# AaltoML/free-hunch

Measured on AMD Instinct MI355X. Metric: images/sec (256x256, num_steps=30, FH-Heun), higher is better.
Workload: dtype f32 UNet (convolutions: exact 3-way bf16 split on the bf16 MFMA, fp32 accuracy) + f64 covariance/CG; 1 GPU; FFHQ-256 arch, gaussian_blur, FH low-rank covariance (dct_diagonal), num_steps=30 heun, batch=8 per GPU; lockstep_groups_per_gpu=2, unet_backend=hip, net_calls_per_image=59

## Files before the change

### free-hunch_amd/_lib.py

```python
from __future__ import annotations

import ctypes as C
import os

import torch

_HERE = os.path.dirname(os.path.abspath(__file__))
LIB_PATH = os.path.join(_HERE, "libfh_hip.so")

c_dp = C.c_void_p


class FhProblem(C.Structure):
    _fields_ = [("op", C.c_int32), ("use_dct", C.c_int32), ("planes", C.c_int32), ("stride", C.c_int32),
                ("ntaps", C.c_int32), ("m", C.c_int32), ("ldm", C.c_int32), ("halo", C.c_int32),
                ("d", C.c_int64), ("sigma_y2", C.c_double),
                ("tap_dy", c_dp), ("tap_dx", c_dp), ("tap_w", c_dp), ("mask", c_dp),
                ("D", c_dp), ("r", c_dp), ("B", c_dp), ("M", c_dp),
                ("ntaps2", C.c_int32), ("halo2", C.c_int32), ("cg_scipy", C.c_int32), ("fold_sym", C.c_int32),
                ("tap2_dy", c_dp), ("tap2_dx", c_dp), ("tap2_w", c_dp),
                ("fold_fwd_w", c_dp), ("fold_fwd_h", c_dp), ("fold_inv_w", c_dp), ("fold_inv_h", c_dp)]


FH_MAX_BATCH = 16
# ... 19 lines not shown
    _fields_ = [("niter", C.c_int32), ("optimal", C.c_int32), ("residual_norm", C.c_double),
                ("b_norm", C.c_double)]


_SIGS = {
    "fh_version": ([], C.c_int),
    "fh_context_create": ([C.POINTER(C.c_void_p), C.c_int, C.c_int, C.c_int], C.c_int),
    "fh_context_destroy": ([C.c_void_p], C.c_int),
    "fh_context_set_exclusive": ([C.c_void_p, C.c_int], C.c_int),
    "fh_context_status": ([C.c_void_p, C.c_void_p], C.c_int),
    "fh_debug_read_stamps": ([C.c_void_p, C.POINTER(C.c_ulonglong), C.c_int, C.c_void_p], C.c_int),
    "fh_dct2d": ([C.c_void_p, c_dp, c_dp, C.c_int, C.c_int, C.c_void_p], C.c_int),
    "fh_dct_sym_plan": ([C.c_int, C.c_int] + [C.POINTER(C.c_int)] * 4 + [C.POINTER(C.c_int64)], C.c_int),
    "fh_dct_rect": ([C.c_void_p, c_dp, c_dp, c_dp, c_dp, C.c_int, C.c_int, C.c_int, C.c_void_p], C.c_int),
    "fh_dct_rect_plan": ([C.c_int] * 4 + [C.POINTER(C.c_int32)], C.c_int),
    "fh_dct_moments_u8": ([C.c_void_p, c_dp, C.c_int, c_dp, c_dp, c_dp, C.c_void_p], C.c_int),
    "fh_rep_apply": ([C.c_void_p, c_dp, c_dp, c_dp, c_dp, C.c_int, c_dp, c_dp, C.c_int64, C.c_int, C.c_void_p], C.c_int),
    "fh_rep_apply_batched": ([C.c_void_p, C.POINTER(FhBatch), C.c_int, c_dp, c_dp, C.c_int64, C.c_int, C.c_void_p], C.c_int),
    "fh_rep_invert": ([C.c_void_p, c_dp, c_dp, c_dp, C.c_double, c_dp, c_dp, c_dp, C.c_int, C.c_int64, C.c_int,
                       C.c_void_p], C.c_int),
    "fh_space_prep": ([C.c_void_p, c_dp, C.c_double, c_dp, c_dp, c_dp, C.c_int64, C.c_void_p], C.c_int),
    "fh_dot": ([C.c_void_p, c_dp, c_dp, c_dp, C.c_int, C.c_int64, C.c_void_p], C.c_int),
    "fh_space_commit": ([C.c_void_p, c_dp, c_dp, C.c_double, C.c_double, C.c_double, c_dp, c_dp, c_dp, c_dp, c_dp,
                         c_dp, c_dp, c_dp, C.c_int, C.c_int64, C.c_void_p], C.c_int),
    "fh_space_commit_dev": ([C.c_void_p, c_dp, c_dp, c_dp, C.c_double, c_dp, c_dp, c_dp, c_dp, c_dp, c_dp, c_dp, c_dp,
                             c_dp, C.c_int, C.c_int, c_dp, C.c_int, C.c_int, C.c_int, C.c_int64, C.c_void_p], C.c_int),
    "fh_cov_time_update": ([C.c_void_p, C.POINTER(FhCovState), c_dp, c_dp, C.c_double, C.c_double, C.c_double, C.c_int,
                            c_dp, c_dp, c_dp, c_dp, C.c_void_p], C.c_int),
    "fh_cov_space_update": ([C.c_void_p, C.POINTER(FhCovState), c_dp, c_dp, C.c_double, c_dp, c_dp, C.c_void_p], C.c_int),
    "fh_cov_time_update_batched": ([C.c_void_p, C.c_int, C.POINTER(FhCovState), c_dp, c_dp, C.c_double, C.c_double, C.c_double,
                                    c_dp, c_dp, c_dp, C.c_void_p], C.c_int),
    "fh_cov_space_update_batched": ([C.c_void_p, C.c_int, C.POINTER(FhCovState), c_dp, c_dp, C.c_double, c_dp, c_dp, c_dp,
                                     C.c_void_p], C.c_int),
    "fh_woodbury_inner": ([C.c_void_p, c_dp, C.c_int, c_dp, C.c_int, c_dp, C.c_int, C.c_int, C.c_void_p], C.c_int),
    "fh_axpby": ([C.c_double, c_dp, C.c_double, c_dp, c_dp, C.c_int64, C.c_void_p], C.c_int),
    "fh_read_scalars": ([C.c_void_p, c_dp, C.POINTER(C.c_double), C.c_int, C.c_void_p], C.c_int),
    "fh_conv_circ": ([C.c_void_p, c_dp, c_dp, c_dp, c_dp, c_dp, C.c_int, C.c_int, C.c_int, C.c_int, C.c_int,
                      C.c_void_p], C.c_int),
    "fh_conv_circ_plan": ([C.c_int] * 6 + [C.POINTER(C.c_int32)], C.c_int),
    "fh_conv_window": ([C.c_void_p, c_dp, c_dp, c_dp, C.c_int, C.c_int, C.c_int, C.c_int, C.c_void_p], C.c_int),
    "fh_conv_window_plan": ([C.c_int] * 4 + [C.POINTER(C.c_int32)], C.c_int),
    "fh_channel_mix": ([C.c_void_p, c_dp, c_dp, c_dp, C.c_int, C.c_int, C.c_void_p], C.c_int),
    "fh_amm": ([C.c_void_p, C.POINTER(FhProblem), c_dp, c_dp, C.c_void_p], C.c_int),
    "fh_dense_matvec_scratch_doubles": ([C.c_int, C.c_int64], C.c_int64),
    "fh_dense_matvec": ([c_dp, c_dp, c_dp, c_dp, C.c_int, C.c_int64, C.c_int, C.c_double, C.c_double, C.c_void_p], C.c_int),
    "fh_dense_rank2": ([c_dp, c_dp, C.c_int, C.c_int64, c_dp, c_dp, c_dp, c_dp, c_dp, c_dp, C.c_double, C.c_double,
                        C.c_void_p], C.c_int),
    "fh_conv2d_nhwc": ([c_dp, c_dp, c_dp, c_dp, c_dp, c_dp] + [C.c_int] * 10 + [C.c_void_p], C.c_int),
    "fh_conv2d_x6_nhwc": ([c_dp, c_dp, c_dp, c_dp, c_dp, c_dp] + [C.c_int] * 10 + [C.c_void_p], C.c_int),
    "fh_conv2d_x6_nhwc_gn": ([c_dp, c_dp, c_dp, c_dp, c_dp, c_dp] + [C.c_int] * 10 + [C.POINTER(FhGnEpilogue), C.c_void_p],
                             C.c_int),
    "fh_conv2d_x6_gn_chunks": ([C.c_int] * 10, C.c_int),
    "fh_conv2d_x6_plan": ([C.c_int] * 10 + [C.POINTER(C.c_int32)], C.c_int),
    "fh_groupnorm_finalize": ([c_dp, c_dp, C.c_int, C.c_int, C.c_double, C.c_int, C.c_void_p], C.c_int),
    "fh_groupnorm_bwd_table": ([c_dp, c_dp, c_dp, c_dp, c_dp, C.c_int, c_dp, C.c_int, C.c_int, C.c_void_p], C.c_int),
    "fh_groupnorm_bwd_apply": ([c_dp] * 8 + [C.c_int, c_dp] + [C.c_int] * 5 + [C.c_void_p], C.c_int),
    "fh_groupnorm_bwd_sums": ([c_dp] * 7 + [C.c_int, c_dp, c_dp] + [C.c_int] * 4 + [C.c_void_p], C.c_int),
    "fh_groupnorm_bwd_apply_ex": ([c_dp] * 8 + [C.c_int, c_dp, c_dp, c_dp, c_dp] + [C.c_int] * 5 + [c_dp, C.c_void_p], C.c_int),
    "fh_groupnorm_small_supported": ([C.c_int, C.c_int], C.c_int),
    "fh_groupnorm_fwd_small": ([c_dp] * 5 + [C.c_int, c_dp, c_dp] + [C.c_int] * 4 + [C.c_void_p], C.c_int),
    "fh_groupnorm_bwd_small": ([c_dp] * 8 + [C.c_int, c_dp, c_dp, c_dp, c_dp] + [C.c_int] * 5 + [C.c_void_p], C.c_int),
    "fh_conv2d_splitk": ([C.c_int] * 7, C.c_int),
    "fh_unet_set_precision": ([C.c_int], C.c_int),
    "fh_unet_get_precision": ([], C.c_int),
    "fh_absmax_f32": ([c_dp, C.c_int64, c_dp, C.c_void_p], C.c_int),
    "fh_groupnorm_table": ([c_dp, c_dp, c_dp, c_dp, c_dp, C.c_int, c_dp, C.c_int, C.c_int, C.c_void_p], C.c_int),
    "fh_conv2d_x6_norm_supported": ([C.c_int] * 5, C.c_int),
    "fh_conv2d_x6_norm_nhwc": ([c_dp, c_dp, C.c_int, c_dp, c_dp, c_dp, c_dp] + [C.c_int] * 5 + [C.c_void_p], C.c_int),
    "fh_conv2d_x6_norm_nhwc_gn": ([c_dp, c_dp, C.c_int, c_dp, c_dp, c_dp, c_dp] + [C.c_int] * 5
                                  + [C.POINTER(FhGnEpilogue), C.c_void_p], C.c_int),
    "fh_conv3x3_thin_nhwc": ([c_dp, c_dp, c_dp, c_dp] + [C.c_int] * 5 + [C.c_void_p], C.c_int),
    "fh_conv3x3_wino_nhwc": ([c_dp, c_dp, c_dp, c_dp, c_dp] + [C.c_int] * 5 + [C.c_void_p], C.c_int),
    "fh_bgemm_f32": ([c_dp, c_dp, c_dp] + [C.c_int] * 10 + [C.c_int64] * 6 + [C.c_float, C.c_void_p], C.c_int),
    "fh_groupnorm_scratch_doubles": ([C.c_int, C.c_int], C.c_int64),
    "fh_groupnorm_stats": ([c_dp, c_dp, c_dp, C.c_int, C.c_int, C.c_int, C.c_void_p], C.c_int),
    "fh_groupnorm_apply": ([c_dp] * 6 + [C.c_int, c_dp, C.c_int, C.c_int, C.c_int, C.c_int, C.c_void_p], C.c_int),
    "fh_groupnorm_bwd": ([c_dp] * 7 + [C.c_int, c_dp, c_dp, c_dp] + [C.c_int] * 5 + [C.c_void_p], C.c_int),
    "fh_attention_supported": ([C.c_int] * 3, C.c_int),
    "fh_attention_fwd": ([c_dp, c_dp, c_dp] + [C.c_int] * 5 + [C.c_void_p], C.c_int),
    "fh_attention_bwd": ([c_dp] * 6 + [C.c_int] * 5 + [C.c_void_p], C.c_int),
    "fh_softmax_rows": ([c_dp, C.c_int64, C.c_int, C.c_void_p], C.c_int),
    "fh_softmax_bwd_rows": ([c_dp, c_dp, C.c_int64, C.c_int, C.c_void_p], C.c_int),
    "fh_resample2x": ([c_dp, c_dp] + [C.c_int] * 5 + [C.c_void_p], C.c_int),
    "fh_concat_channels": ([c_dp, c_dp, c_dp, C.c_int64, C.c_int, C.c_int, C.c_int, C.c_void_p], C.c_int),
    "fh_layout_nchw_nhwc": ([c_dp, c_dp, C.c_int, C.c_int, C.c_int64, C.c_int, C.c_int, C.c_void_p], C.c_int),
    "fh_add_f32": ([c_dp, c_dp, c_dp, C.c_int64, C.c_void_p], C.c_int),
    "fh_metrics_scratch_doubles": ([C.c_int] * 4, C.c_int64),
    "fh_metrics_u8": ([c_dp, c_dp, C.c_int, C.c_int, C.c_int, C.c_int, c_dp, c_dp, c_dp, C.c_void_p], C.c_int),
    "fh_lpips_prep_u8": ([c_dp, c_dp, c_dp, c_dp, C.c_int, C.c_int, C.c_int, C.c_void_p], C.c_int),
    "fh_relu_f32": ([c_dp, C.c_int64, C.c_void_p], C.c_int),
    "fh_relu_maxpool2_nhwc": ([c_dp, c_dp, C.c_int, C.c_int, C.c_int, C.c_int, C.c_void_p], C.c_int),
    "fh_lpips_tap_scratch_doubles": ([C.c_int], C.c_int64),
    "fh_lpips_tap": ([c_dp, c_dp, C.c_int, C.c_int, C.c_int, C.c_int, c_dp, c_dp, C.c_int, C.c_void_p], C.c_int),
    "fh_noisy_u8": ([c_dp, C.POINTER(C.c_int64), C.c_int, C.c_int, C.c_double, C.c_int, C.c_uint64, c_dp, C.c_void_p], C.c_int),
    "fh_sqerr_u8_scratch_doubles": ([C.c_int, C.c_int], C.c_int64),
    "fh_sqerr_u8": ([c_dp, c_dp, C.c_int, C.c_int, c_dp, c_dp, C.c_void_p], C.c_int),
    "fh_cg_solve_batched": ([C.c_void_p, C.POINTER(FhProblem), C.POINTER(FhBatch), c_dp, c_dp, C.POINTER(C.c_double),
                             C.c_double, C.c_int, C.POINTER(FhCgInfo), C.c_void_p], C.c_int),
    "fh_cg_solve": ([C.c_void_p, C.POINTER(FhProblem), c_dp, c_dp, C.c_double, C.c_double, C.c_int,
                     C.POINTER(FhCgInfo), C.c_void_p], C.c_int),
}

_lib = None


class FhError(RuntimeError):
# ... 134 lines not shown
```

### free-hunch_amd/csrc/fh_unet.hip

```cpp
#include "fh_common.h"
#include <stdlib.h>

typedef float float16_t __attribute__((ext_vector_type(16)));

namespace {

constexpr int kBK = 32;
constexpr int kLd = kBK + 4;

struct ConvArgs {
  const float* in;
  const float* w;
  const float* bias;
  const float* res;
  float* out;
  int N, H, W, Cin, Cout, KH, KW, pad, stride, Ho, Wo;
  int ksplit;
  float* ws;
};

__device__ __forceinline__ void xcd_tile(int& tile_m, int& tile_n) {
  const unsigned gx = gridDim.x, gy = gridDim.y;
  const unsigned total = gx * gy;
  unsigned lin = blockIdx.y * gx + blockIdx.x;
// ... 235 lines not shown
    a.gn_partial[((int64_t)n * a.gn_chunks + chunk) * 64 + tid] = sum;
  }
}

__device__ __forceinline__ void split3(float x, __bf16& h, __bf16& m, __bf16& l) {
  h = (__bf16)x;
  float r = x - (float)h;
  m = (__bf16)r;
  r -= (float)m;
  l = (__bf16)r;
}

typedef _Float16 f16x8_t __attribute__((ext_vector_type(8)));
__device__ __forceinline__ __bf16 half_bits(float x) {
  const _Float16 h = (_Float16)x;
  return __builtin_bit_cast(__bf16, h);
}
template <bool F16>
__device__ __forceinline__ float16_t mfma16(bf16x8_t a, bf16x8_t b, float16_t c) {
  if (F16) return __builtin_amdgcn_mfma_f32_32x32x16_f16(__builtin_bit_cast(f16x8_t, a), __builtin_bit_cast(f16x8_t, b), c, 0, 0, 0);
  return __builtin_amdgcn_mfma_f32_32x32x16_bf16(a, b, c, 0, 0, 0);
}

struct SplitScale {
  float in, inv_in, winv;
};
template <int NP, bool F16>
__device__ __forceinline__ SplitScale split_scale(const ConvArgsX& a, int64_t wplane) {
  SplitScale s{1.f, 1.f, 1.f};
  if (F16 && NP == 2) {
    s.winv = *reinterpret_cast<const float*>(a.wx + 2 * wplane);
    if (a.in_amax != nullptr) {
      unsigned mb = 0u;
#pragma unroll
      for (int q = 0; q < FH_AMAX_SLOTS; ++q) mb = max(mb, __float_as_uint(a.in_amax[q]));
      int e = (int)((mb >> 23) & 255u) - 127;
      e = e < -110 ? -110 : (e > 126 ? 126 : e);
      s.in = __uint_as_float((unsigned)(127 + 11 - e) << 23);
      s.inv_in = __uint_as_float((unsigned)(127 - 11 + e) << 23);
    } else {
      s.in = a.in_scale;
      s.inv_in = 1.f / a.in_scale;
    }
  }
  return s;
}
__device__ __forceinline__ void split_half2(float xs, __bf16& h, __bf16& m) {
  xs = fminf(fmaxf(xs, -65504.f), 65504.f);
  const _Float16 hh = (_Float16)xs;
  h = __builtin_bit_cast(__bf16, hh);
  m = half_bits(xs - (float)hh);
}

template <int MI, int NI, int WM, int WN, int MINW, int NP = 3, bool F16 = false>
__global__ __launch_bounds__(64 * WM * WN, MINW) void k_conv_x6(ConvArgsX a) {
  constexpr int T = 64 * WM * WN;
  constexpr int BM = WM * MI * 32, BN = WN * NI * 32;
  constexpr int IA = BM * 8 / T;
  constexpr int IB = (NP * BN * 4 + T - 1) / T;
  static_assert(BM * 8 % T == 0, "tile / thread-count mismatch");
  __shared__ __align__(16) __bf16 As[NP][BM][kXLd];
  __shared__ __align__(16) __bf16 Bs[NP][BN][kXLd];

  const int tid = threadIdx.x, lane = tid & 63, wave = tid >> 6;
  const int wm = (wave / WN) * (MI * 32), wn = (wave % WN) * (NI * 32);
  const int lr = lane & 31, lh = lane >> 5;
  const int64_t M = (int64_t)a.N * a.Ho * a.Wo;
  int tile_m, tile_n;
  xcd_tile(tile_m, tile_n);
  const int64_t m0 = (int64_t)tile_m * BM;
  const int n0 = tile_n * BN;
  const int taps = a.KH * a.KW;
  const int cpt = a.Cin / kBK;
  const int nchunks_all = taps * cpt;
  const int c_begin = (int)((int64_t)nchunks_all * blockIdx.z / a.ksplit);
  const int c_end = (int)((int64_t)nchunks_all * (blockIdx.z + 1) / a.ksplit);

  int a_row[IA], a_n[IA], a_ho[IA], a_wo[IA];
  bool a_ok[IA];
  const int a_c4 = (tid & 7) * 4;
#pragma unroll
  for (int e = 0; e < IA; ++e) {
    a_row[e] = (e * T + tid) >> 3;
    const int64_t pm = m0 + a_row[e];
    a_ok[e] = pm < M;
    a_n[e] = a_ho[e] = a_wo[e] = 0;
    if (a_ok[e]) {
      a_n[e] = (int)(pm / ((int64_t)a.Ho * a.Wo));
      const int rem = (int)(pm % ((int64_t)a.Ho * a.Wo));
      a_ho[e] = rem / a.Wo;
      a_wo[e] = rem % a.Wo;
    }
  }
  const int64_t wplane = (int64_t)taps * cpt * a.Cout * kBK;
  const SplitScale ssc = split_scale<NP, F16>(a, wplane);
  int b_pl[IB], b_row[IB];
  bool b_ok[IB];
  const int b_part = (tid & 3) * 8;
#pragma unroll
  for (int e = 0; e < IB; ++e) {
    const int idx = e * T + tid;
    b_pl[e] = idx < NP * BN * 4 ? idx / (BN * 4) : -1;
    b_row[e] = (idx % (BN * 4)) >> 2;
    b_ok[e] = b_pl[e] >= 0 && n0 + b_row[e] < a.Cout;
  }

  float4 ra_reg[IA];
  bf16x8_t rb_reg[IB];

  auto load_chunk = [&](int c) {
    const int cc = c / taps, tap = c % taps;
    const int ky = tap / a.KW, kx = tap % a.KW;
#pragma unroll
    for (int e = 0; e < IA; ++e) {
      const int hi = a_ho[e] * a.stride + ky - a.pad, wi = a_wo[e] * a.stride + kx - a.pad;
      const bool ok = a_ok[e] && hi >= 0 && hi < a.H && wi >= 0 && wi < a.W;
      const float* src = a.in + (((int64_t)a_n[e] * a.H + (ok ? hi : 0)) * a.W + (ok ? wi : 0)) * a.Cin + cc * kBK + a_c4;
      ra_reg[e] = ok ? *reinterpret_cast<const float4*>(src) : make_float4(0.f, 0.f, 0.f, 0.f);
    }
    const __bf16* wbase = a.wx + ((int64_t)tap * cpt + cc) * a.Cout * kBK;
#pragma unroll
    for (int e = 0; e < IB; ++e) {
      bf16x8_t z;
#pragma unroll
      for (int q = 0; q < 8; ++q) z[q] = (__bf16)0.f;
      const __bf16* src = wbase + (b_ok[e] ? b_pl[e] : 0) * wplane + (int64_t)(b_ok[e] ? n0 + b_row[e] : 0) * kBK + b_part;
      rb_reg[e] = b_ok[e] ? *reinterpret_cast<const bf16x8_t*>(src) : z;
    }
  };
  typedef __bf16 bf16x4_t __attribute__((ext_vector_type(4)));
  auto store_chunk = [&]() {
#pragma unroll
    for (int e = 0; e < IA; ++e) {
      bf16x4_t h4, m4, l4;
      const float4 v = ra_reg[e];
#pragma unroll
      for (int q = 0; q < 4; ++q) {
        const float x = q == 0 ? v.x : q == 1 ? v.y : q == 2 ? v.z : v.w;
        __bf16 h, m, l;
        if (F16 && NP == 2) {
          split_half2(x * ssc.in, h, m);
          l = m;
        } else {
          split3(x, h, m, l);
          if (F16) h = half_bits(x);
        }
        h4[q] = h, m4[q] = m, l4[q] = l;
      }
      *reinterpret_cast<bf16x4_t*>(&As[0][a_row[e]][a_c4]) = h4;
      if (NP >= 2) *reinterpret_cast<bf16x4_t*>(&As[NP >= 2 ? 1 : 0][a_row[e]][a_c4]) = m4;
      if (NP == 3) *reinterpret_cast<bf16x4_t*>(&As[NP - 1][a_row[e]][a_c4]) = l4;
    }
#pragma unroll
    for (int e = 0; e < IB; ++e)
      if (b_pl[e] >= 0) *reinterpret_cast<bf16x8_t*>(&Bs[b_pl[e]][b_row[e]][b_part]) = rb_reg[e];
  };

  float16_t acc[MI][NI];
#pragma unroll
  for (int i = 0; i < MI; ++i)
#pragma unroll
    for (int j = 0; j < NI; ++j)
#pragma unroll
      for (int r = 0; r < 16; ++r) acc[i][j][r] = 0.f;

  auto compute = [&]() {
#pragma unroll
  for (int ks = 0; ks < kBK / 16; ++ks) {
    const int ko = ks * 16 + 8 * lh;
    bf16x8_t af[NP][MI], bfr[NP][NI];
#pragma unroll
    for (int p = 0; p < NP; ++p) {
#pragma unroll
      for (int i = 0; i < MI; ++i) af[p][i] = *reinterpret_cast<const bf16x8_t*>(&As[p][wm + i * 32 + lr][ko]);
#pragma unroll
      for (int j = 0; j < NI; ++j) bfr[p][j] = *reinterpret_cast<const bf16x8_t*>(&Bs[p][wn + j * 32 + lr][ko]);
    }
#pragma unroll
    for (int i = 0; i < MI; ++i)
#pragma unroll
      for (int j = 0; j < NI; ++j) {
        float16_t t = acc[i][j];
        if (NP == 3) {
          t = __builtin_amdgcn_mfma_f32_32x32x16_bf16(af[NP - 1][i], bfr[0][j], t, 0, 0, 0);
          t = __builtin_amdgcn_mfma_f32_32x32x16_bf16(af[0][i], bfr[NP - 1][j], t, 0, 0, 0);
          t = __builtin_amdgcn_mfma_f32_32x32x16_bf16(af[NP >= 2 ? 1 : 0][i], bfr[NP >= 2 ? 1 : 0][j], t, 0, 0, 0);
        }
        if (NP >= 2) {
          t = mfma16<F16>(af[NP >= 2 ? 1 : 0][i], bfr[0][j], t);
          t = mfma16<F16>(af[0][i], bfr[NP >= 2 ? 1 : 0][j], t);
        }
        t = mfma16<F16>(af[0][i], bfr[0][j], t);
        acc[i][j] = t;
      }
  }
  };

  load_chunk(c_begin);
  store_chunk();
  __syncthreads();
  for (int c = c_begin; c < c_end; ++c) {
    if (c + 1 < c_end) load_chunk(c + 1);
    compute();
    __syncthreads();
    if (c + 1 < c_end) {
      store_chunk();
      __syncthreads();
    }
  }

  __shared__ double gred[WM * WN * 32 * NI * 2];
  const bool gn = a.gn_partial != nullptr;
  const int gn_n = gn ? (int)(m0 / ((int64_t)a.Ho * a.Wo)) : 0;
  GnAcc gsum[NI];
#pragma unroll
  for (int j = 0; j < NI; ++j) {
    gsum[j].s0 = gsum[j].s1 = 0.f;
    const int co = n0 + wn + j * 32 + lr;
    if (co >= a.Cout) continue;
    const float bv = (a.bias != nullptr && a.ksplit == 1) ? a.bias[co] : 0.f;
    float* dst = a.ksplit == 1 ? a.out : a.ws + (int64_t)blockIdx.z * M * a.Cout;
    float tb[5] = {0.f, 0.f, 0.f, 0.f, 0.f};
    if (gn && a.gn_mode == 1) {
#pragma unroll
      for (int q = 0; q < 5; ++q) tb[q] = a.gn_tab[((int64_t)gn_n * 5 + q) * a.Cout + co];
    }
#pragma unroll
    for (int i = 0; i < MI; ++i) {
#pragma unroll
      for (int r = 0; r < 16; ++r) {
        const int64_t row = m0 + wm + i * 32 + (r & 3) + 8 * (r >> 2) + 4 * lh;
        if (row < M) {
          float v = acc[i][j][r];
          if (F16 && NP == 2) v = v * ssc.inv_in * ssc.winv;
          v += bv;
          if (a.res != nullptr && a.ksplit == 1) v += a.res[row * a.Cout + co];
          dst[row * a.Cout + co] = v;
          if (gn) gn_accum(a, gsum[j], v, row, co, tb);
        }
      }
    }
  }
  if (gn) {
    const int tiles_per_img = (int)(((int64_t)a.Ho * a.Wo) / BM);
    gn_reduce<NI, WM, WN, BN>(a, gsum, gred, gn_n, (tile_m % tiles_per_img) * (int)gridDim.y + tile_n, n0);
  }
}

template <int SEGW, bool NORM = false, int BM = 128, int NP = 3, int GL = 0, bool F16 = false, bool SPLIT = false, bool TT = false>
__global__ __launch_bounds__(4 * BM, 4) void k_conv_x6r(ConvArgsX a) {
  static_assert(!SPLIT || (GL == 0 && BM == 128 && !NORM), "split-K: the register-staged 128-pixel tile, plain input");
  static_assert(!TT || (GL == 1 && BM == 256 && NP == 3 && !F16 && !SPLIT), "tile tail: the exact-split 256-pixel tile");
  constexpr int MI = 2, NI = 1, WN = 4, T = 4 * BM;
  constexpr int NSEG = BM / SEGW, SP = SEGW + 2;
  constexpr int BN = 128, AR = NSEG * SP;
  constexpr int IA = (AR * 8 + T - 1) / T;
  constexpr int IB = (NP * BN * 4 + T - 1) / T;
  constexpr int NB = GL == 2 ? 3 : (GL ? 2 : 1);
  constexpr int NA = GL == 2 ? 2 : 1;
// ... 1211 lines not shown
                                                int64_t P, int Ca, int Cb, int split) {
  const int C4 = (Ca + Cb) / 4, Ca4 = Ca / 4, Cb4 = Cb / 4;
  for (int64_t i = (int64_t)blockIdx.x * 256 + threadIdx.x; i < P * C4; i += (int64_t)gridDim.x * 256) {
    const int c4 = (int)(i % C4);
    const int64_t p = i / C4;
    float4* o = reinterpret_cast<float4*>(out) + i;
    float4* s = c4 < Ca4 ? reinterpret_cast<float4*>(a) + p * Ca4 + c4 : reinterpret_cast<float4*>(b) + p * Cb4 + (c4 - Ca4);
    if (split) *s = *o; else *o = *s;
  }
}

__global__ __launch_bounds__(256) void k_nchw_to_nhwc(const float* __restrict__ in, float* __restrict__ out, int N,
                                                      int C, int64_t P, int Cp) {
  for (int64_t i = (int64_t)blockIdx.x * 256 + threadIdx.x; i < (int64_t)N * P * Cp; i += (int64_t)gridDim.x * 256) {
    const int c = (int)(i % Cp);
    const int64_t p = (i / Cp) % P, n = i / (Cp * P);
    out[i] = c < C ? in[((int64_t)n * C + c) * P + p] : 0.f;
  }
}
__global__ __launch_bounds__(256) void k_nhwc_to_nchw(const float* __restrict__ in, float* __restrict__ out, int N,
                                                      int C, int64_t P, int Cp) {
  for (int64_t i = (int64_t)blockIdx.x * 256 + threadIdx.x; i < (int64_t)N * C * P; i += (int64_t)gridDim.x * 256) {
    const int64_t p = i % P;
    const int c = (int)((i / P) % C);
    const int64_t n = i / (P * C);
    out[i] = in[((int64_t)n * P + p) * Cp + c];
  }
}

__global__ __launch_bounds__(256) void k_add_f32(const float* __restrict__ a, const float* __restrict__ b,
                                                 float* __restrict__ out, int64_t n4) {
  for (int64_t i = (int64_t)blockIdx.x * 256 + threadIdx.x; i < n4; i += (int64_t)gridDim.x * 256) {
    const float4 x = reinterpret_cast<const float4*>(a)[i], y = reinterpret_cast<const float4*>(b)[i];
    reinterpret_cast<float4*>(out)[i] = make_float4(x.x + y.x, x.y + y.y, x.z + y.z, x.w + y.w);
  }
}

inline unsigned grid_for(int64_t work_items, int per_block = 256, int cap = 4096) {
  int64_t b = (work_items + per_block - 1) / per_block;
  return (unsigned)(b < 1 ? 1 : (b > cap ? cap : b));
}

thread_local int g_conv_np = 3;

struct X6Plan {
  bool reuse;
  int bm, bn;
  int segw;
  int gl;
  bool split;
  dim3 grid, block;
  bool norm;
  int gn_bm;
};

bool splitk_reuse_enabled() {
  static const bool on = !(getenv("FH_CONV_SPLITK_REUSE") != nullptr && atoi(getenv("FH_CONV_SPLITK_REUSE")) == 0);
  return on;
}

X6Plan x6_plan(int ksplit, int N, int H, int W, int , int Cout, int KH, int KW, int pad,
               int stride, bool norm) {
  const int Ho = (H + 2 * pad - KH) / stride + 1, Wo = (W + 2 * pad - KW) / stride + 1;
  const int64_t M = (int64_t)N * Ho * Wo;
  const int nb128 = (Cout + 127) / 128;
  const int64_t b128 = ((M + 127) / 128) * nb128;
  X6Plan p{};
  p.bn = 128, p.norm = norm;
  if (ksplit == 1 && Cout > 64 && b128 >= 384) {
    const bool r3 = KH == 3 && KW == 3 && pad == 1 && stride == 1 && M % 128 == 0;
    const bool big = r3 && M % 256 == 0 && (M / 256) * nb128 >= 256;
    p.reuse = true;
    if (big && W % 256 == 0)
      p.bm = 256, p.segw = 256;
    else if (big && W == 128 && H % 2 == 0)
      p.bm = 256, p.segw = 128;
    else if (big && W == 64 && H % 4 == 0)
      p.bm = 256, p.segw = 64;
    else if (r3 && W % 128 == 0)
      p.bm = 128, p.segw = 128;
    else if (r3 && W == 64 && H % 2 == 0)
      p.bm = 128, p.segw = 64;
    else if (r3 && W == 32 && H % 4 == 0)
      p.bm = 128, p.segw = 32;
    else
      p.reuse = false, p.bm = 128;
    p.gl = p.bm == 256;
  } else if (ksplit > 1 && Cout > 64 && b128 * ksplit >= 256) {
    p.bm = 128;
    const bool r3 = KH == 3 && KW == 3 && pad == 1 && stride == 1 && ((int64_t)H * W) % 128 == 0 && splitk_reuse_enabled();
    if (r3 && W % 128 == 0)
      p.reuse = p.split = true, p.segw = 128;
    else if (r3 && W == 64 && H % 2 == 0)
      p.reuse = p.split = true, p.segw = 64;
    else if (r3 && W == 32 && H % 4 == 0)
      p.reuse = p.split = true, p.segw = 32;
    else if (r3 && W == 16 && H % 8 == 0)
      p.reuse = p.split = true, p.segw = 16;
  } else if (ksplit == 1 && Cout > 64 && ((M + 63) / 64) * nb128 >= 256) {
    p.bm = 64;
  } else {
    p.bm = 64, p.bn = 64;
  }
  p.grid = dim3((unsigned)((M + p.bm - 1) / p.bm), (unsigned)((Cout + p.bn - 1) / p.bn), (unsigned)ksplit);
  p.block = dim3(p.reuse ? 4 * p.bm : (p.bm == 128 ? 512 : 256));
  p.gn_bm = (ksplit == 1 && Cout > 64 && p.bn == 128 && Cout % 32 == 0 && (Ho * Wo) % p.bm == 0) ? p.bm : 0;
  return p;
}

bool conv_tile_tail_enabled() {
  static const bool on = !(getenv("FH_CONV_TILE_TAIL") != nullptr && atoi(getenv("FH_CONV_TILE_TAIL")) == 0);
  return on;
}

template <int SEGW, bool NORM, int BM, int GL, bool SPLIT = false>
void launch_x6r(const X6Plan& p, hipStream_t st, const ConvArgsX& a) {
  switch (g_conv_np) {
    case 1: hipLaunchKernelGGL((k_conv_x6r<SEGW, NORM, BM, 1, GL, false, SPLIT>), p.grid, p.block, 0, st, a); break;
    case 2: hipLaunchKernelGGL((k_conv_x6r<SEGW, NORM, BM, 2, GL, false, SPLIT>), p.grid, p.block, 0, st, a); break;
    case 16: hipLaunchKernelGGL((k_conv_x6r<SEGW, NORM, BM, 1, GL, true, SPLIT>), p.grid, p.block, 0, st, a); break;
    case 32: hipLaunchKernelGGL((k_conv_x6r<SEGW, NORM, BM, 2, GL == 1 ? 2 : GL, true, SPLIT>), p.grid, p.block, 0, st, a); break;
    default: hipLaunchKernelGGL((k_conv_x6r<SEGW, NORM, BM, 3, GL, false, SPLIT>), p.grid, p.block, 0, st, a); break;
  }
}

template <int MI, int NI, int WM, int WN, int MINW>
void launch_x6(const X6Plan& p, hipStream_t st, const ConvArgsX& a) {
  switch (g_conv_np) {
    case 1: hipLaunchKernelGGL((k_conv_x6<MI, NI, WM, WN, MINW, 1>), p.grid, p.block, 0, st, a); break;
    case 2: hipLaunchKernelGGL((k_conv_x6<MI, NI, WM, WN, MINW, 2>), p.grid, p.block, 0, st, a); break;
    case 16: hipLaunchKernelGGL((k_conv_x6<MI, NI, WM, WN, MINW, 1, true>), p.grid, p.block, 0, st, a); break;
    case 32: hipLaunchKernelGGL((k_conv_x6<MI, NI, WM, WN, MINW, 2, true>), p.grid, p.block, 0, st, a); break;
    default: hipLaunchKernelGGL((k_conv_x6<MI, NI, WM, WN, MINW, 3>), p.grid, p.block, 0, st, a); break;
  }
}

constexpr int tile_key(int bm, int w, int gl = 0) { return (bm * 1024 + w) * 2 + gl; }

template <int SEGW, bool NORM>
void launch_x6r_256(const X6Plan& p, hipStream_t st, const ConvArgsX& a) {
  if (g_conv_np == 3 && conv_tile_tail_enabled())
    hipLaunchKernelGGL((k_conv_x6r<SEGW, NORM, 256, 3, 1, false, false, true>), p.grid, p.block, 0, st, a);
  else
    launch_x6r<SEGW, NORM, 256, 1>(p, st, a);
}

template <bool NORM>
bool launch_x6r_tile(const X6Plan& p, hipStream_t st, const ConvArgsX& a) {
  switch (tile_key(p.bm, p.segw, p.gl)) {
    case tile_key(256, 256, 1): launch_x6r_256<256, NORM>(p, st, a); return true;
    case tile_key(256, 128, 1): launch_x6r_256<128, NORM>(p, st, a); return true;
    case tile_key(256, 64, 1): launch_x6r_256<64, NORM>(p, st, a); return true;
    case tile_key(128, 128, 0): launch_x6r<128, NORM, 128, 0>(p, st, a); return true;
    case tile_key(128, 64, 0): launch_x6r<64, NORM, 128, 0>(p, st, a); return true;
    case tile_key(128, 32, 0): launch_x6r<32, NORM, 128, 0>(p, st, a); return true;
  }
  return false;
}

bool launch_x6r_split_tile(const X6Plan& p, hipStream_t st, const ConvArgsX& a) {
  if (p.norm || p.bm != 128 || p.gl != 0) return false;
  switch (p.segw) {
    case 128: launch_x6r<128, false, 128, 0, true>(p, st, a); return true;
    case 64: launch_x6r<64, false, 128, 0, true>(p, st, a); return true;
    case 32: launch_x6r<32, false, 128, 0, true>(p, st, a); return true;
    case 16: launch_x6r<16, false, 128, 0, true>(p, st, a); return true;
  }
  return false;
}

bool launch_x6_tile(const X6Plan& p, hipStream_t st, const ConvArgsX& a) {
  switch (tile_key(p.bm, p.bn)) {
    case tile_key(128, 128): launch_x6<2, 1, 2, 4, 4>(p, st, a); return true;
    case tile_key(64, 128): launch_x6<1, 2, 2, 2, 2>(p, st, a); return true;
    case tile_key(64, 64): launch_x6<1, 1, 2, 2, 2>(p, st, a); return true;
  }
  return false;
}

}

extern "C" {

int fh_unet_set_precision(int mode) {
  if (mode < 0 || mode > 4) return FH_EINVAL;
  g_conv_np = mode == 0 ? 3 : (mode == 1 ? 1 : (mode == 2 ? 2 : (mode == 3 ? 16 : 32)));
  return 0;
}

int fh_unet_get_precision(void) {
  return g_conv_np == 3 ? 0 : (g_conv_np == 1 ? 1 : (g_conv_np == 2 ? 2 : (g_conv_np == 16 ? 3 : 4)));
}

int fh_absmax_f32(const float* x, int64_t n, float* out, void* stream) {
  if (!out || n < 0 || (n > 0 && !x) || ((uintptr_t)x & 15)) return FH_EINVAL;
  hipStream_t st = (hipStream_t)stream;
  FH_CHECK(hipMemsetAsync(out, 0, FH_AMAX_SLOTS * sizeof(float), st));
  if (n > 0) {
    const int64_t want = (n / 4 + 255) / 256;
    hipLaunchKernelGGL(k_absmax, dim3((unsigned)(want < 1 ? 1 : (want > 2048 ? 2048 : want))), dim3(256), 0, st, x, n,
                       reinterpret_cast<unsigned*>(out));
  }
  FH_LAUNCH_CHECK();
  return 0;
}

int fh_conv2d_splitk(int N, int Ho, int Wo, int Cin, int Cout, int KH, int KW) {
  const int64_t M = (int64_t)N * Ho * Wo;
  const int64_t blocks = ((M + 63) / 64) * ((Cout + 63) / 64);
  const int nchunks = KH * KW * (Cin / kBK);
  int z = 1;
  constexpr int target = 2048;
  constexpr int zmax = 8;
  while (blocks * z < target && z < zmax && nchunks / (2 * z) >= 6) z *= 2;
  return z;
}

int fh_conv2d_nhwc(const float* in, const float* w, const float* bias, const float* res, float* out, float* ws,
                   int ksplit, int N, int H, int W, int Cin, int Cout, int KH, int KW, int pad, int stride,
                   void* stream) {
  if (!in || !w || !out || N < 1 || H < 1 || W < 1 || Cin < kBK || Cin % kBK != 0 || Cout < 1 || stride < 1)
    return FH_EINVAL;
  if (ksplit < 1 || ksplit > 32 || (ksplit > 1 && !ws)) return FH_EINVAL;
  ConvArgs a;
  a.in = in, a.w = w, a.bias = bias, a.res = res, a.out = out;
  a.N = N, a.H = H, a.W = W, a.Cin = Cin, a.Cout = Cout, a.KH = KH, a.KW = KW, a.pad = pad, a.stride = stride;
  a.Ho = (H + 2 * pad - KH) / stride + 1;
  a.Wo = (W + 2 * pad - KW) / stride + 1;
  a.ksplit = ksplit, a.ws = ws;
  const int64_t M = (int64_t)N * a.Ho * a.Wo;
  hipStream_t st = (hipStream_t)stream;
  const unsigned Z = (unsigned)ksplit;
  const int64_t b128 = ((M + 127) / 128) * ((Cout + 127) / 128);
  if (ksplit == 1 && Cout > 64 && b128 >= 384) {
    hipLaunchKernelGGL((k_conv_igemm<2, 2>), dim3((unsigned)((M + 127) / 128), (Cout + 127) / 128, 1), dim3(256), 0, st, a);
  } else if (ksplit == 1 && Cout > 64 && ((M + 63) / 64) * ((Cout + 127) / 128) >= 256) {
    hipLaunchKernelGGL((k_conv_igemm<1, 2>), dim3((unsigned)((M + 63) / 64), (Cout + 127) / 128, 1), dim3(256), 0, st, a);
  } else {
    hipLaunchKernelGGL((k_conv_igemm<1, 1>), dim3((unsigned)((M + 63) / 64), (Cout + 63) / 64, Z), dim3(256), 0, st, a);
  }
  if (ksplit > 1) {
    const int64_t total = M * Cout;
    hipLaunchKernelGGL(k_splitk_reduce, dim3(grid_for(total)), dim3(256), 0, st, (const float*)ws, bias, res, out, total,
                       Cout, ksplit);
  }
  FH_LAUNCH_CHECK();
  return 0;
}

int fh_conv2d_x6_gn_chunks(int ksplit, int N, int H, int W, int Cin, int Cout, int KH, int KW, int pad, int stride) {
  if (N < 1 || H < 1 || W < 1 || Cout < 1 || stride < 1) return 0;
  const X6Plan p = x6_plan(ksplit, N, H, W, Cin, Cout, KH, KW, pad, stride, false);
  const int Ho = (H + 2 * pad - KH) / stride + 1, Wo = (W + 2 * pad - KW) / stride + 1;
  return p.gn_bm ? (Ho * Wo / p.gn_bm) * ((Cout + 127) / 128) : 0;
}

int fh_conv2d_x6_plan(int ksplit, int N, int H, int W, int Cin, int Cout, int KH, int KW, int pad, int stride,
                      int32_t* plan) {
  if (!plan || N < 1 || H < 1 || W < 1 || Cin < kBK || Cin % kBK != 0 || Cout < 1 || stride < 1 || ksplit < 1 || ksplit > 32)
    return FH_EINVAL;
  const X6Plan p = x6_plan(ksplit, N, H, W, Cin, Cout, KH, KW, pad, stride, false);
  plan[0] = !p.reuse ? 0 : (p.split ? 2 : 1);
  plan[1] = p.bm, plan[2] = p.bn, plan[3] = p.reuse ? p.segw : 0, plan[4] = p.reuse ? p.gl : 0;
  plan[5] = (int32_t)p.grid.x, plan[6] = (int32_t)p.grid.y, plan[7] = (int32_t)p.grid.z;
  return 0;
}

#ifdef FH_CONV_PHASE_CLOCKS
static unsigned long long* g_phase_buf = nullptr;
int fh_conv_phase_buffer(void* buf) {
  g_phase_buf = (unsigned long long*)buf;
  return 0;
}
#endif

static int set_gn(ConvArgsX& a, const fh_gn_epilogue* epi, int chunks) {
  a.gn_partial = nullptr, a.gn_x = nullptr, a.gn_tab = nullptr, a.gn_mode = a.gn_act = a.gn_chunks = 0;
  a.in_amax = epi != nullptr ? epi->in_amax : nullptr, a.in_scale = 1.f;
  if (g_conv_np == 32 && a.ab == nullptr && a.in_amax == nullptr) return FH_EINVAL;
  if (a.ab != nullptr) a.in_amax = nullptr, a.in_scale = 16.f;
  if (epi == nullptr || epi->partial == nullptr) return 0;
  if (chunks <= 0 || epi->mode < 0 || epi->mode > 1 || (epi->mode == 1 && (!epi->x || !epi->tab))) return FH_EINVAL;
  a.gn_partial = epi->partial, a.gn_x = epi->x, a.gn_tab = epi->tab;
  a.gn_mode = epi->mode, a.gn_act = epi->act, a.gn_chunks = chunks;
  return 0;
}

static int conv2d_x6_launch(const float* in, bool norm, const float* ab_table, int act, const void* wx, const float* bias,
                            const float* res, float* out, float* ws, int ksplit, int N, int H, int W, int Cin, int Cout,
                            int KH, int KW, int pad, int stride, const fh_gn_epilogue* epi, void* stream) {
  if (!in || !wx || !out || N < 1 || H < 1 || W < 1 || Cin < kBK || Cin % kBK != 0 || Cout < 1 || stride < 1)
    return FH_EINVAL;
  if (ksplit < 1 || ksplit > 32 || (ksplit > 1 && !ws)) return FH_EINVAL;
  const X6Plan p = x6_plan(ksplit, N, H, W, Cin, Cout, KH, KW, pad, stride, norm);
  if (norm && (!ab_table || !p.reuse)) return FH_EINVAL;
  ConvArgsX a;
  a.ab = norm ? ab_table : nullptr, a.act = norm ? act : 0;
  a.in = in, a.wx = (const __bf16*)wx, a.bias = bias, a.res = res, a.out = out;
  a.N = N, a.H = H, a.W = W, a.Cin = Cin, a.Cout = Cout, a.KH = KH, a.KW = KW, a.pad = pad, a.stride = stride;
  a.Ho = (H + 2 * pad - KH) / stride + 1;
  a.Wo = (W + 2 * pad - KW) / stride + 1;
  a.ksplit = ksplit, a.ws = ws;
  {
    const int rc = set_gn(a, epi, p.gn_bm ? (a.Ho * a.Wo / p.gn_bm) * ((Cout + 127) / 128) : 0);
    if (rc) return rc;
  }
#ifdef FH_CONV_PHASE_CLOCKS
  a.phase = g_phase_buf;
#endif
  a.wide = Cout % 4 == 0 && (((uintptr_t)out | (uintptr_t)res | (uintptr_t)a.gn_x) & 15) == 0;
  hipStream_t st = (hipStream_t)stream;
  const bool built = !p.reuse ? launch_x6_tile(p, st, a)
                     : p.split ? launch_x6r_split_tile(p, st, a)
                     : p.norm ? launch_x6r_tile<true>(p, st, a)
                              : launch_x6r_tile<false>(p, st, a);
  if (!built) return FH_ESIZE;
  if (ksplit > 1) {
    const int64_t total = (int64_t)N * a.Ho * a.Wo * Cout;
    hipLaunchKernelGGL(k_splitk_reduce, dim3(grid_for(total)), dim3(256), 0, st, (const float*)ws, bias, res, out, total,
                       Cout, ksplit);
// ... 285 lines not shown
```

### include/fh_hip.h

```cpp
#ifndef FH_HIP_H
#define FH_HIP_H

#include <stdint.h>

#ifdef __cplusplus
extern "C" {
#endif

#define FH_EINVAL (-1)
#define FH_ESYNC (-3)
#define FH_ESIZE (-2)
#define FH_MAX_COLS 256

typedef struct fh_context fh_context;

int fh_version(void);
int fh_context_create(fh_context** out, int S, int planes_max, int m_cap);
int fh_context_destroy(fh_context* ctx);
int fh_context_set_exclusive(fh_context* ctx, int exclusive);
int fh_context_status(fh_context* ctx, void* stream);
int fh_debug_read_stamps(fh_context* ctx, unsigned long long* out_host, int count, void* stream);

int fh_dct2d(fh_context* ctx, const double* in, double* out, int planes, int inverse, void* stream);

// ... 108 lines not shown
  const double* D[FH_MAX_BATCH];
  const double* r[FH_MAX_BATCH];
  const double* B[FH_MAX_BATCH];
  const double* M[FH_MAX_BATCH];
  const double* mask[FH_MAX_BATCH];
} fh_batch;

typedef struct fh_cg_info {
  int32_t niter;
  int32_t optimal;
  double residual_norm;
  double b_norm;
} fh_cg_info;

int fh_rep_apply_batched(fh_context* ctx, const fh_batch* per, int ldm, const double* z, double* out, int64_t d, int m,
                         void* stream);

int fh_amm(fh_context* ctx, const fh_problem* p, const double* u, double* out, void* stream);
int fh_cg_solve(fh_context* ctx, const fh_problem* p, const double* b, double* x, double rtol, double atol,
                int maxiter, fh_cg_info* info_host, void* stream);
int fh_cg_solve_batched(fh_context* ctx, const fh_problem* shared, const fh_batch* per, const double* b, double* x,
                        const double* rtol_host, double atol, int maxiter, fh_cg_info* info_host, void* stream);


int fh_conv2d_nhwc(const float* in, const float* w, const float* bias, const float* res, float* out, float* ws,
                   int ksplit, int N, int H, int W, int Cin, int Cout, int KH, int KW, int pad, int stride,
                   void* stream);
int fh_unet_set_precision(int mode);
int fh_unet_get_precision(void);
#define FH_AMAX_SLOTS 16
int fh_absmax_f32(const float* x, int64_t n, float* out, void* stream);
int fh_conv2d_splitk(int N, int Ho, int Wo, int Cin, int Cout, int KH, int KW);

int fh_conv2d_x6_nhwc(const float* in, const void* wx, const float* bias, const float* res, float* out, float* ws,
                      int ksplit, int N, int H, int W, int Cin, int Cout, int KH, int KW, int pad, int stride,
                      void* stream);

int fh_groupnorm_table(const float* stats, const float* gamma, const float* beta, const float* scale, const float* shift,
                       int ss_stride, float* table, int N, int C, void* stream);
int fh_conv2d_x6_norm_supported(int N, int H, int W, int Cin, int Cout);
int fh_conv2d_x6_norm_nhwc(const float* in, const float* ab_table, int act, const void* wx, const float* bias,
                           const float* res, float* out, int N, int H, int W, int Cin, int Cout, void* stream);

typedef struct fh_gn_epilogue {
  double* partial;
  const float* x;
  const float* tab;
  int32_t mode, act;
  const float* in_amax;
} fh_gn_epilogue;
int fh_conv2d_x6_gn_chunks(int ksplit, int N, int H, int W, int Cin, int Cout, int KH, int KW, int pad, int stride);
int fh_conv2d_x6_plan(int ksplit, int N, int H, int W, int Cin, int Cout, int KH, int KW, int pad, int stride,
                      int32_t* plan);
int fh_conv2d_x6_nhwc_gn(const float* in, const void* wx, const float* bias, const float* res, float* out, float* ws,
                         int ksplit, int N, int H, int W, int Cin, int Cout, int KH, int KW, int pad, int stride,
                         const fh_gn_epilogue* epi, void* stream);
int fh_conv2d_x6_norm_nhwc_gn(const float* in, const float* ab_table, int act, const void* wx, const float* bias,
                              const float* res, float* out, int N, int H, int W, int Cin, int Cout, const fh_gn_epilogue* epi,
                              void* stream);
int fh_groupnorm_finalize(const double* partial, float* out, int N, int chunks, double count, int mode, void* stream);
int fh_groupnorm_bwd_table(const float* stats, const float* gamma, const float* beta, const float* scale, const float* shift,
                           int ss_stride, float* table, int N, int C, void* stream);
int fh_groupnorm_bwd_apply(const float* x, const float* dy, const float* stats, const float* sums, const float* gamma,
                           const float* beta, const float* scale, const float* shift, int ss_stride, float* dx, int N, int P,
                           int C, int act, int accumulate, void* stream);
int fh_groupnorm_bwd_sums(const float* x, const float* dy, const float* stats, const float* gamma, const float* beta,
                          const float* scale, const float* shift, int ss_stride, float* sums, double* scratch, int N, int P,
                          int C, int act, void* stream);
int fh_groupnorm_bwd_apply_ex(const float* x, const float* dy, const float* stats, const float* sums, const float* gamma,
                              const float* beta, const float* scale, const float* shift, int ss_stride, const float* acc_src,
                              const float* add2, float* dx, float* dx2, int csplit, int N, int P, int C, int act, float* amax2,
                              void* stream);

int fh_groupnorm_small_supported(int P, int C);
int fh_groupnorm_fwd_small(const float* x, const float* gamma, const float* beta, const float* scale, const float* shift,
                           int ss_stride, float* y, float* stats, int N, int P, int C, int act, void* stream);
int fh_groupnorm_bwd_small(const float* x, const float* dy, const float* stats, float* sums, const float* gamma,
                           const float* beta, const float* scale, const float* shift, int ss_stride, const float* acc_src,
                           const float* add2, float* dx, float* dx2, int csplit, int N, int P, int C, int act, void* stream);

int fh_conv3x3_thin_nhwc(const float* in, const float* w, const float* bias, float* out, int N, int H, int W, int Cin,
                         int Cout, void* stream);

int fh_conv3x3_wino_nhwc(const float* in, const float* wu, const float* bias, const float* res, float* out, int N,
                         int H, int W, int Cin, int Cout, void* stream);

int fh_bgemm_f32(const float* A, const float* B, float* C, int M, int N, int K, int lda, int ldb, int ldc, int transA,
                 int transB, int batch, int inner, int64_t sA0, int64_t sA1, int64_t sB0, int64_t sB1, int64_t sC0,
                 int64_t sC1, float alpha, void* stream);

int64_t fh_groupnorm_scratch_doubles(int N, int P);
int fh_groupnorm_stats(const float* x, float* stats, double* scratch, int N, int P, int C, void* stream);
int fh_groupnorm_apply(const float* x, const float* stats, const float* gamma, const float* beta, const float* scale,
                       const float* shift, int ss_stride, float* y, int N, int P, int C, int act, void* stream);
int fh_groupnorm_bwd(const float* x, const float* dy, const float* stats, const float* gamma, const float* beta,
                     const float* scale, const float* shift, int ss_stride, float* sums, double* scratch, float* dx, int N,
                     int P, int C, int act, int accumulate, void* stream);

int fh_softmax_rows(float* s, int64_t rows, int T, void* stream);
int fh_softmax_bwd_rows(const float* p, float* dp, int64_t rows, int T, void* stream);

int fh_attention_supported(int T, int C, int heads);
int fh_attention_fwd(const float* qkv, float* out, float* lse, int N, int T, int C, int heads, int new_order, void* stream);
int fh_attention_bwd(const float* qkv, const float* out, const float* dout, const float* lse, float* dsum, float* dqkv, int N,
                     int T, int C, int heads, int new_order, void* stream);

// ... 36 lines not shown
```

Baseline: 2.594 images/s.

## Process two K-chunks per barrier in 64x64 x6 conv tiles for small grids

Adds a template depth G to the x6 implicit-GEMM conv kernel so each pipeline stage loads, splits and computes G K-chunks between barriers, with G-deep shared-memory and register staging. Depth 2 is used for 64x64 tiles when the grid has at most 256 workgroups, with an env override and a query function that reports depth and shared-memory size. The aim is to halve barrier count and expose more memory-level parallelism in latency-bound small convolutions, at the cost of doubled LDS and register use, which lowers occupancy.

```diff
diff --git a/free-hunch_amd/_lib.py b/free-hunch_amd/_lib.py
--- a/free-hunch_amd/_lib.py
+++ b/free-hunch_amd/_lib.py
@@ -95,6 +95,7 @@
                              C.c_int),
     "fh_conv2d_x6_gn_chunks": ([C.c_int] * 10, C.c_int),
     "fh_conv2d_x6_plan": ([C.c_int] * 10 + [C.POINTER(C.c_int32)], C.c_int),
+    "fh_conv2d_x6_depth": ([C.c_int] * 10 + [C.POINTER(C.c_int32)], C.c_int),
     "fh_groupnorm_finalize": ([c_dp, c_dp, C.c_int, C.c_int, C.c_double, C.c_int, C.c_void_p], C.c_int),
     "fh_groupnorm_bwd_table": ([c_dp, c_dp, c_dp, c_dp, c_dp, C.c_int, c_dp, C.c_int, C.c_int, C.c_void_p], C.c_int),
     "fh_groupnorm_bwd_apply": ([c_dp] * 8 + [C.c_int, c_dp] + [C.c_int] * 5 + [C.c_void_p], C.c_int),
diff --git a/free-hunch_amd/csrc/fh_unet.hip b/free-hunch_amd/csrc/fh_unet.hip
--- a/free-hunch_amd/csrc/fh_unet.hip
+++ b/free-hunch_amd/csrc/fh_unet.hip
@@ -311,15 +311,15 @@
   m = half_bits(xs - (float)hh);
 }
 
-template <int MI, int NI, int WM, int WN, int MINW, int NP = 3, bool F16 = false>
+template <int MI, int NI, int WM, int WN, int MINW, int NP = 3, bool F16 = false, int G = 1>
 __global__ __launch_bounds__(64 * WM * WN, MINW) void k_conv_x6(ConvArgsX a) {
   constexpr int T = 64 * WM * WN;
   constexpr int BM = WM * MI * 32, BN = WN * NI * 32;
   constexpr int IA = BM * 8 / T;
   constexpr int IB = (NP * BN * 4 + T - 1) / T;
   static_assert(BM * 8 % T == 0, "tile / thread-count mismatch");
-  __shared__ __align__(16) __bf16 As[NP][BM][kXLd];
-  __shared__ __align__(16) __bf16 Bs[NP][BN][kXLd];
+  __shared__ __align__(16) __bf16 As[G][NP][BM][kXLd];
+  __shared__ __align__(16) __bf16 Bs[G][NP][BN][kXLd];
 
   const int tid = threadIdx.x, lane = tid & 63, wave = tid >> 6;
   const int wm = (wave / WN) * (MI * 32), wn = (wave % WN) * (NI * 32);
@@ -364,10 +364,14 @@
     b_ok[e] = b_pl[e] >= 0 && n0 + b_row[e] < a.Cout;
   }
 
-  float4 ra_reg[IA];
-  bf16x8_t rb_reg[IB];
-
-  auto load_chunk = [&](int c) {
+  float4 ra_reg[G][IA];
+  bf16x8_t rb_reg[G][IB];
+
+  auto load_chunk = [&](int c0) {
+#pragma unroll
+   for (int g = 0; g < G; ++g) {
+    const int c = c0 + g;
+    if (G > 1 && c >= c_end) break;
     const int cc = c / taps, tap = c % taps;
     const int ky = tap / a.KW, kx = tap % a.KW;
 #pragma unroll
@@ -375,7 +379,7 @@
       const int hi = a_ho[e] * a.stride + ky - a.pad, wi = a_wo[e] * a.stride + kx - a.pad;
       const bool ok = a_ok[e] && hi >= 0 && hi < a.H && wi >= 0 && wi < a.W;
       const float* src = a.in + (((int64_t)a_n[e] * a.H + (ok ? hi : 0)) * a.W + (ok ? wi : 0)) * a.Cin + cc * kBK + a_c4;
-      ra_reg[e] = ok ? *reinterpret_cast<const float4*>(src) : make_float4(0.f, 0.f, 0.f, 0.f);
+      ra_reg[g][e] = ok ? *reinterpret_cast<const float4*>(src) : make_float4(0.f, 0.f, 0.f, 0.f);
     }
     const __bf16* wbase = a.wx + ((int64_t)tap * cpt + cc) * a.Cout * kBK;
 #pragma unroll
@@ -384,15 +388,19 @@
 #pragma unroll
       for (int q = 0; q < 8; ++q) z[q] = (__bf16)0.f;
       const __bf16* src = wbase + (b_ok[e] ? b_pl[e] : 0) * wplane + (int64_t)(b_ok[e] ? n0 + b_row[e] : 0) * kBK + b_part;
-      rb_reg[e] = b_ok[e] ? *reinterpret_cast<const bf16x8_t*>(src) : z;
-    }
+      rb_reg[g][e] = b_ok[e] ? *reinterpret_cast<const bf16x8_t*>(src) : z;
+    }
+   }
   };
   typedef __bf16 bf16x4_t __attribute__((ext_vector_type(4)));
-  auto store_chunk = [&]() {
+  auto store_chunk = [&](int c0) {
+#pragma unroll
+   for (int g = 0; g < G; ++g) {
+    if (G > 1 && c0 + g >= c_end) break;
 #pragma unroll
     for (int e = 0; e < IA; ++e) {
       bf16x4_t h4, m4, l4;
-      const float4 v = ra_reg[e];
+      const float4 v = ra_reg[g][e];
 #pragma unroll
       for (int q = 0; q < 4; ++q) {
         const float x = q == 0 ? v.x : q == 1 ? v.y : q == 2 ? v.z : v.w;
@@ -406,13 +414,14 @@
         }
         h4[q] = h, m4[q] = m, l4[q] = l;
       }
-      *reinterpret_cast<bf16x4_t*>(&As[0][a_row[e]][a_c4]) = h4;
-      if (NP >= 2) *reinterpret_cast<bf16x4_t*>(&As[NP >= 2 ? 1 : 0][a_row[e]][a_c4]) = m4;
-      if (NP == 3) *reinterpret_cast<bf16x4_t*>(&As[NP - 1][a_row[e]][a_c4]) = l4;
+      *reinterpret_cast<bf16x4_t*>(&As[g][0][a_row[e]][a_c4]) = h4;
+      if (NP >= 2) *reinterpret_cast<bf16x4_t*>(&As[g][NP >= 2 ? 1 : 0][a_row[e]][a_c4]) = m4;
+      if (NP == 3) *reinterpret_cast<bf16x4_t*>(&As[g][NP - 1][a_row[e]][a_c4]) = l4;
     }
 #pragma unroll
     for (int e = 0; e < IB; ++e)
-      if (b_pl[e] >= 0) *reinterpret_cast<bf16x8_t*>(&Bs[b_pl[e]][b_row[e]][b_part]) = rb_reg[e];
+      if (b_pl[e] >= 0) *reinterpret_cast<bf16x8_t*>(&Bs[g][b_pl[e]][b_row[e]][b_part]) = rb_reg[g][e];
+   }
   };
 
   float16_t acc[MI][NI];
@@ -423,7 +432,10 @@
 #pragma unroll
       for (int r = 0; r < 16; ++r) acc[i][j][r] = 0.f;
 
-  auto compute = [&]() {
+  auto compute = [&](int c0) {
+#pragma unroll
+ for (int g = 0; g < G; ++g) {
+  if (G > 1 && c0 + g >= c_end) break;
 #pragma unroll
   for (int ks = 0; ks < kBK / 16; ++ks) {
     const int ko = ks * 16 + 8 * lh;
@@ -431,9 +443,9 @@
 #pragma unroll
     for (int p = 0; p < NP; ++p) {
 #pragma unroll
-      for (int i = 0; i < MI; ++i) af[p][i] = *reinterpret_cast<const bf16x8_t*>(&As[p][wm + i * 32 + lr][ko]);
-#pragma unroll
-      for (int j = 0; j < NI; ++j) bfr[p][j] = *reinterpret_cast<const bf16x8_t*>(&Bs[p][wn + j * 32 + lr][ko]);
+      for (int i = 0; i < MI; ++i) af[p][i] = *reinterpret_cast<const bf16x8_t*>(&As[g][p][wm + i * 32 + lr][ko]);
+#pragma unroll
+      for (int j = 0; j < NI; ++j) bfr[p][j] = *reinterpret_cast<const bf16x8_t*>(&Bs[g][p][wn + j * 32 + lr][ko]);
     }
 #pragma unroll
     for (int i = 0; i < MI; ++i)
@@ -453,17 +465,18 @@
         acc[i][j] = t;
       }
   }
+ }
   };
 
   load_chunk(c_begin);
-  store_chunk();
+  store_chunk(c_begin);
   __syncthreads();
-  for (int c = c_begin; c < c_end; ++c) {
-    if (c + 1 < c_end) load_chunk(c + 1);
-    compute();
+  for (int c = c_begin; c < c_end; c += G) {
+    if (c + G < c_end) load_chunk(c + G);
+    compute(c);
     __syncthreads();
-    if (c + 1 < c_end) {
-      store_chunk();
+    if (c + G < c_end) {
+      store_chunk(c + G);
       __syncthreads();
     }
   }
@@ -1781,11 +1794,24 @@
   dim3 grid, block;
   bool norm;
   int gn_bm;
+  int depth;
 };
 
 bool splitk_reuse_enabled() {
   static const bool on = !(getenv("FH_CONV_SPLITK_REUSE") != nullptr && atoi(getenv("FH_CONV_SPLITK_REUSE")) == 0);
   return on;
+}
+
+constexpr int64_t kDepth2MaxWg = 256;
+
+int conv_depth_switch() {
+  static const int v = getenv("FH_CONV_DEPTH") != nullptr ? atoi(getenv("FH_CONV_DEPTH")) : 0;
+  return v;
+}
+
+int x6_depth(int bm, int bn, int64_t workgroups) {
+  if (bm != 64 || bn != 64 || conv_depth_switch() == 1) return 1;
+  return (conv_depth_switch() == 2 || workgroups <= kDepth2MaxWg) ? 2 : 1;
 }
 
 X6Plan x6_plan(int ksplit, int N, int H, int W, int , int Cout, int KH, int KW, int pad,
@@ -1834,6 +1860,7 @@
   p.grid = dim3((unsigned)((M + p.bm - 1) / p.bm), (unsigned)((Cout + p.bn - 1) / p.bn), (unsigned)ksplit);
   p.block = dim3(p.reuse ? 4 * p.bm : (p.bm == 128 ? 512 : 256));
   p.gn_bm = (ksplit == 1 && Cout > 64 && p.bn == 128 && Cout % 32 == 0 && (Ho * Wo) % p.bm == 0) ? p.bm : 0;
+  p.depth = p.reuse ? 1 : x6_depth(p.bm, p.bn, (int64_t)p.grid.x * p.grid.y * p.grid.z);
   return p;
 }
 
@@ -1899,6 +1926,11 @@
 }
 
 bool launch_x6_tile(const X6Plan& p, hipStream_t st, const ConvArgsX& a) {
+  if (g_conv_np == 3 && p.depth > 1) {
+    if (p.bm != 64 || p.bn != 64 || p.depth != 2) return false;
+    hipLaunchKernelGGL((k_conv_x6<1, 1, 2, 2, 2, 3, false, 2>), p.grid, p.block, 0, st, a);
+    return true;
+  }
   switch (tile_key(p.bm, p.bn)) {
     case tile_key(128, 128): launch_x6<2, 1, 2, 4, 4>(p, st, a); return true;
     case tile_key(64, 128): launch_x6<1, 2, 2, 2, 2>(p, st, a); return true;
@@ -1995,6 +2027,25 @@
   return 0;
 }
 
+int fh_conv2d_x6_depth(int ksplit, int N, int H, int W, int Cin, int Cout, int KH, int KW, int pad, int stride,
+                       int32_t* out) {
+  if (!out || N < 1 || H < 1 || W < 1 || Cin < kBK || Cin % kBK != 0 || Cout < 1 || stride < 1 || ksplit < 1 || ksplit > 32)
+    return FH_EINVAL;
+  const X6Plan p = x6_plan(ksplit, N, H, W, Cin, Cout, KH, KW, pad, stride, false);
+  const int np = g_conv_np == 3 ? 3 : ((g_conv_np == 2 || g_conv_np == 32) ? 2 : 1);
+  out[0] = g_conv_np == 3 ? p.depth : 1;
+  if (!p.reuse) {
+    const int waves = p.bm == 128 ? 8 : 4, ni = p.bm == 64 && p.bn == 128 ? 2 : 1;
+    out[1] = out[0] * np * (p.bm + p.bn) * kXLd * 2 + waves * 32 * ni * 2 * 8;
+  } else {
+    const int gl = (p.gl == 1 && g_conv_np == 32) ? 2 : p.gl;
+    const int ar = (p.bm / p.segw) * (p.segw + 2);
+    out[1] = (gl == 2 ? 2 : 1) * np * ar * kXLd * 2 + (gl == 2 ? 3 : (gl ? 2 : 1)) * np * 128 * (gl ? kBK : kXLd) * 2 +
+             (p.bm / 64) * 4 * 32 * 2 * 8;
+  }
+  return 0;
+}
+
 #ifdef FH_CONV_PHASE_CLOCKS
 static unsigned long long* g_phase_buf = nullptr;
 int fh_conv_phase_buffer(void* buf) {
diff --git a/include/fh_hip.h b/include/fh_hip.h
--- a/include/fh_hip.h
+++ b/include/fh_hip.h
@@ -184,6 +184,8 @@
 int fh_conv2d_x6_gn_chunks(int ksplit, int N, int H, int W, int Cin, int Cout, int KH, int KW, int pad, int stride);
 int fh_conv2d_x6_plan(int ksplit, int N, int H, int W, int Cin, int Cout, int KH, int KW, int pad, int stride,
                       int32_t* plan);
+int fh_conv2d_x6_depth(int ksplit, int N, int H, int W, int Cin, int Cout, int KH, int KW, int pad, int stride,
+                       int32_t out[2]);
 int fh_conv2d_x6_nhwc_gn(const float* in, const void* wx, const float* bias, const float* res, float* out, float* ws,
                          int ksplit, int N, int H, int W, int Cin, int Cout, int KH, int KW, int pad, int stride,
                          const fh_gn_epilogue* epi, void* stream);
```

Result: no change. 2.613 images/s (median of 3 runs) (+0.7%).
